# rongzhao-zhang/EfficientQ

Hardware: AMD Instinct MI355X
Metric: ptq_calibration_throughput (higher is better)
Workload: dtype i8xi8->i32 (exact) for the Gram systems and per-iteration loss convs of the layers with quantised input, f32/f64 elsewhere

## Files before the change

efficientq_amd/csrc/admm_run.hip:

```cpp
#include <stdlib.h>
#include <algorithm>
#include <vector>
#include "common.h"
#include "internal.h"
#include "project_dual.h"

namespace effq {

struct ProfRec {
  int kind, iter, loss_kind, c2, n;
  effq_geom geom;
  hipEvent_t e0, e1;
};
static thread_local std::vector<ProfRec> g_prof;
static thread_local int g_prof_every = 0;
enum { PROF_PROX = 1, PROF_FIXED_POINT = 2, PROF_PROJECT = 3, PROF_LOSS = 4, PROF_INVERSE = 5, PROF_WAIT = 6 };

struct ProfScope {
  bool on;
  hipStream_t stream;
  ProfRec rec;
  ProfScope(bool enabled, int kind, int iter, const effq_admm_run_args* a, hipStream_t st) : on(enabled), stream(st) {
    if (!on) return;
    rec.kind = kind;
// ... 239 lines not shown
};

static int enqueue_later_inverses(const effq_admm_run_args* a, const AdmmPlan& p, EventPool& events, hipEvent_t* ev_inv) {
  for (int r = p.first + 1; r < p.rhos.count; ++r) {
    float* dst = a->ainv_pool + (size_t)(r - p.first) * p.ainv_elems;
    const bool on2 = p.two_sides && ((r - p.first) % 2 == 0);
    hipStream_t sr = on2 ? p.s_side2 : p.s_side;
    void* ws = !p.fork_side ? a->inv_ws : (on2 ? a->inv_ws_side2 : a->inv_ws_side);
    const size_t wsb = !p.fork_side ? a->inv_ws_bytes : (on2 ? a->inv_ws_side2_bytes : a->inv_ws_side_bytes);
    ProfScope ps(g_prof_every > 0, PROF_INVERSE, -1 - r, a, sr);
    const int rc = effq_spd_inverse(a->A0, p.n, p.has_b, p.rhos.rho[r], a->eta, dst, ws, wsb, sr);
    if (rc != EFFQ_OK) return rc;
    ps.close();
    if (p.fork_side) {
      EFFQ_HIP(events.take(&ev_inv[r]));
      EFFQ_HIP(hipEventRecord(ev_inv[r], sr));
    }
  }
  return EFFQ_OK;
}

struct AdmmIter {
  int i;
  double rho, rho_next;
  float dual_div;
  bool use_shift, use_traj, prof;
  bool next_rhs;
  const float* G_prev;
  float *G, *bstar;
  int8_t* Gq;
  effq_fp_state* st;
  const float* parts;
  int parts_n, parts_ld;
};
static AdmmIter admm_iter(const effq_admm_run_args* a, const AdmmPlan& p, int i, double rho, bool use_traj) {
  const bool step = i % a->rho_period == 0, doubles = rho * 2 <= a->rho_max;
  const bool use_shift = p.rhos.shifted_first && i == 0;
  const bool prof = g_prof_every > 0 && !use_shift && (i % g_prof_every) == g_prof_every / 2;
  return AdmmIter{i, rho, !step ? rho : doubles ? rho * 2 : a->rho_max,
                  !step ? 1.0f : doubles ? 2.0f : (float)(a->rho_max / rho), use_shift, use_traj, prof, i + 1 < a->iters,
                  (i == 0) ? a->W0 : a->G_ring + (size_t)(i - 1) * p.nw, a->G_ring + (size_t)i * p.nw,
                  p.has_b ? a->b_ring + (size_t)i * p.c2 : nullptr, a->Gq_ring ? a->Gq_ring + (size_t)i * p.nw : nullptr,
                  a->state_ring + i, nullptr, 1, 0};
}

static int enqueue_prox(const effq_admm_run_args* a, const AdmmPlan& p, AdmmIter* it, const float* Ainv, bool bm_ready) {
  if (!it->use_shift && bm_ready && it->use_traj && p.c2 <= 512)
    return effq_prox_solve_prebuilt_parts(a->B0, Ainv, a->W0, a->b0, it->G_prev, a->dual, p.c2, p.n, p.has_b, it->rho,
                                          a->eta, a->wstar, it->bstar, a->prox_ws, a->prox_ws_bytes, p.s_main,
                                          &it->parts, &it->parts_n, &it->parts_ld);
  if (it->use_shift)
    return effq_prox_solve_shifted(a->B0, a->ainv_pool, a->W0, a->b0, it->G_prev, a->dual, p.c2, p.n, p.has_b, it->rho,
                                   a->eta, p.rhos.rho[1], shift_terms(it->rho, a->eta, p.rhos.rho[1]), a->wstar, it->bstar,
                                   a->prox_ws, a->prox_ws_bytes, p.s_main);
  const auto solve = bm_ready ? effq_prox_solve_prebuilt : effq_prox_solve;
  return solve(a->B0, Ainv, a->W0, a->b0, it->G_prev, a->dual, p.c2, p.n, p.has_b, it->rho, a->eta, a->wstar, it->bstar,
               a->prox_ws, a->prox_ws_bytes, p.s_main);
}

enum class FpKind { channels, traj, bucket, small, coop };
static FpKind fp_kind(const AdmmPlan& p, bool use_traj) {
  if (p.chan) return FpKind::channels;
  if (use_traj) return FpKind::traj;
  if (p.bucket) return FpKind::bucket;
  return p.nw <= effq_fp_small_max() ? FpKind::small : FpKind::coop;
}

static int enqueue_fixed_point(const effq_admm_run_args* a, const AdmmPlan& p, const AdmmIter& it, bool* bm_ready) {
  const int nwrow = p.n - p.has_b;
  ProjNext nx;
  memset(&nx, 0, sizeof(nx));
  if (it.next_rhs) nx = ProjNext{p.bm, a->B0, a->W0, nwrow, p.n, p.bm_ld, (float)it.rho_next, (float)a->eta};
  const ProjNext* nxp = it.next_rhs ? &nx : nullptr;
  const FpKind kind = fp_kind(p, it.use_traj);
  const bool fuse_proj = kind == FpKind::channels ||
                         (kind == FpKind::small && proj_vec_ok(a->v, a->wstar, it.G, a->dual, it.Gq, p.nw, nxp));
  ProjFused pf;
  memset(&pf, 0, sizeof(pf));
  pf.wstar = a->wstar; pf.G = it.G; pf.dual = a->dual; pf.Gq = it.Gq; pf.err_flag = a->err_flag;
  pf.d = 2.0 / (double)(a->w_levels - 1); pf.dual_div = it.dual_div; pf.lm1 = a->w_levels - 1;
  pf.n4 = (unsigned)(p.nw / 4);
  pf.nx = nx;
  void* rec = p.traj ? a->fp_pred : nullptr;
  const int maxit = 100 * a->w_levels;
  ProfScope p_fp(it.prof, PROF_FIXED_POINT, it.i, a, p.s_main);
  int rc;
  if (kind == FpKind::channels)
    rc = effq_fixed_point_channels_proj(a->wstar, a->dual, a->v, p.c2, nwrow, a->w_levels, a->tol, maxit,
                                        a->alpha_ring + (size_t)it.i * p.c2,
                                        a->w_iters_ring ? a->w_iters_ring + (size_t)it.i * p.c2 : nullptr, a->err_flag,
                                        it.G, it.dual_div, it.next_rhs ? p.bm : nullptr, a->B0, a->W0, p.n, p.bm_ld,
                                        it.rho_next, a->eta, p.s_main);
  else if (kind == FpKind::traj && it.parts != nullptr)
    rc = effq_fixed_point_traj_parts(it.parts, it.parts_n, it.parts_ld, p.c2, nwrow, p.has_b, a->dual, a->wstar, it.bstar,
                                     a->v, a->w_levels, -1.0, 1.0, a->tol, maxit, it.st, a->fp_pred, a->fp_traj_ws,
                                     a->fp_traj_ws_bytes, p.s_main);
  else if (kind == FpKind::traj)
    rc = effq_fixed_point_traj(a->wstar, a->dual, a->v, p.nw, a->w_levels, -1.0, 1.0, a->tol, maxit, it.st, a->fp_pred,
                               a->fp_traj_ws, a->fp_traj_ws_bytes, p.s_main);
  else if (kind == FpKind::bucket)
    rc = effq_fixed_point_bucket_rec(a->wstar, a->dual, a->v, p.nw, a->w_levels, -1.0, 1.0, a->tol, maxit, it.st, a->fp_ws,
                                     a->fp_ws_bytes, rec, p.s_main);
  else if (kind == FpKind::small)
    rc = effq_fixed_point_small_fused(a->wstar, a->dual, a->v, p.nw, a->w_levels, -1.0, 1.0, a->tol, maxit, it.st,
                                      fuse_proj ? &pf : nullptr, p.s_main);
  else
    rc = effq_fixed_point_coop_rec(a->wstar, a->dual, a->v, p.nw, a->w_levels, -1.0, 1.0, a->tol, maxit, it.st, a->red_ws,
                                   rec, p.s_main);
  if (rc != EFFQ_OK) return rc;
  p_fp.close();
  *bm_ready = it.next_rhs;
  if (fuse_proj) return EFFQ_OK;
  ProfScope p_pr(it.prof, PROF_PROJECT, it.i, a, p.s_main);
  rc = effq_project_dual_impl(a->v, a->wstar, it.st, a->w_levels, it.G, a->dual, it.dual_div, it.Gq, p.nw, a->err_flag,
                              nxp, p.s_main);
  if (rc != EFFQ_OK) return rc;
  p_pr.close();
  return EFFQ_OK;
}

static int enqueue_losses(const effq_admm_run_args* a, const AdmmPlan& p, int j0, int i) {
  const int step = a->loss_kind == 5 ? 16 : 1;
  for (int j = j0; j <= i; j += step) {
    const int cnt = (i - j + 1 < step) ? (i - j + 1) : step;
    const float* Gj = a->G_ring + (size_t)j * p.nw;
    const int8_t* Gqj = a->Gq_ring ? a->Gq_ring + (size_t)j * p.nw : nullptr;
    const float* bj = p.has_b ? a->b_ring + (size_t)j * p.c2 : nullptr;
    const effq_fp_state* stj = a->state_ring + j;
    double* sq = a->hist + 2 * (size_t)j;
    const bool prof = g_prof_every > 0 && (a->loss_kind == 5 ? (j / p.loss_group) % 2 == 1 :
                      !(p.rhos.shifted_first && j == 0) && (j % g_prof_every) == g_prof_every / 2);
    ProfScope p_loss(prof, PROF_LOSS, j, a, p.s_loss);
    int rc;
    if (a->loss_kind == 5)
      rc = effq_gram_loss_i8(a->loss_planes, a->loss_nplanes, a->loss_Au, a->loss_Bu, a->loss_syy, Gqj, bj, stj,
// ... 49 lines not shown
    hipEvent_t ev_fork;
    EFFQ_HIP(events.take(&ev_fork));
    EFFQ_HIP(hipEventRecord(ev_fork, p.s_main));
    EFFQ_HIP(hipStreamWaitEvent(p.s_side, ev_fork, 0));
    if (p.two_sides) EFFQ_HIP(hipStreamWaitEvent(p.s_side2, ev_fork, 0));
  }
  ProfScope p_inv(g_prof_every > 0, PROF_INVERSE, -1, a, p.s_main);
  if (const int rc = effq_spd_inverse(a->A0, p.n, p.has_b, p.rhos.rho[p.first], a->eta, a->ainv_pool, a->inv_ws,
                                      a->inv_ws_bytes, p.s_main); rc != EFFQ_OK)
    return rc;
  p_inv.close();
  if (p.fork_loss)
    for (int e = 0; e < LOSS_EVENTS; ++e) EFFQ_HIP(events.take(&ev_loss[e]));
  bool bm_ready = false;
  const float* Ainv = nullptr;
  int k = 0;
  int cur = -1;
  int loss_next = 0;
  for (int i = 0; i < a->iters; ++i) {
    if (k + 1 < p.rhos.count && p.rhos.first_iter[k + 1] == i) ++k;
    if (i == p.side_iter)
      if (const int rc = enqueue_later_inverses(a, p, events, ev_inv); rc != EFFQ_OK) return rc;
    AdmmIter it = admm_iter(a, p, i, p.rhos.rho[k], p.traj && i - p.rhos.first_iter[k] >= p.traj_after);
    if (!it.use_shift && cur != k) {
      EFFQ_CHECK_ARG(p.rhos.rho[k] == p.rhos.rho[k]);
      if (p.fork_side && ev_inv[k] != nullptr) {
        ProfScope p_wait(g_prof_every > 0, PROF_WAIT, i, a, p.s_main);
        EFFQ_HIP(hipStreamWaitEvent(p.s_main, ev_inv[k], 0));
        p_wait.close();
      }
      Ainv = a->ainv_pool + (size_t)(k - p.first) * p.ainv_elems;
      cur = k;
    }
    ProfScope p_prox(it.prof, PROF_PROX, i, a, p.s_main);
    if (const int rc = enqueue_prox(a, p, &it, Ainv, bm_ready); rc != EFFQ_OK) return rc;
    p_prox.close();
    if (const int rc = enqueue_fixed_point(a, p, it, &bm_ready); rc != EFFQ_OK) return rc;
    if (a->res_ring != nullptr) {
      const size_t nb = std::min<size_t>((p.nw + 1023) / 1024, 256);
      hipLaunchKernelGGL(k_admm_residuals, dim3((unsigned)nb), dim3(256), 0, p.s_main, a->wstar, it.G, it.G_prev, p.nw,
                         a->res_ring + 2 * (size_t)i);
      EFFQ_LAUNCH_CHECK();
    }
    if (!p.fork_loss || (i + 1) % p.loss_group == 0 || i + 1 == a->iters) {
      if (p.fork_loss) EFFQ_HIP(events.hand_over(p.s_main, p.s_loss, ev_loss[(i / p.loss_group) % LOSS_EVENTS]));
      if (const int rc = enqueue_losses(a, p, loss_next, i); rc != EFFQ_OK) return rc;
      loss_next = i + 1;
    }
  }
  ProfScope p_join(g_prof_every > 0 && (p.fork_loss || p.fork_side), PROF_WAIT, a->iters, a, p.s_main);
  if (p.fork_loss) EFFQ_HIP(events.hand_over(p.s_loss, p.s_main));
  if (p.fork_side && p.n_inv > 1) EFFQ_HIP(events.hand_over(p.s_side, p.s_main));
  if (p.fork_side && p.n_inv > 1 && p.two_sides) EFFQ_HIP(events.hand_over(p.s_side2, p.s_main));
  p_join.close();
  return EFFQ_OK;
}

size_t effq_gram_packed_elems(int n, int c2) {
  return (n > 0 && c2 > 0) ? (size_t)n * (n + 1) / 2 + (size_t)c2 * n : 0;
}

int effq_gram_pack(const float* A0, const float* B0, int n, int c2, float* buf, void* stream) {
  EFFQ_CHECK_ARG(A0 && B0 && buf && n > 0 && c2 > 0);
  size_t blocks = ((size_t)n * n + (size_t)c2 * n + 255) / 256;
  if (blocks > 8192) blocks = 8192;
  hipLaunchKernelGGL(k_gram_pack, dim3((unsigned)blocks), dim3(256), 0, as_stream(stream), A0, B0, n, c2, buf);
  EFFQ_LAUNCH_CHECK();
  return EFFQ_OK;
}
// ... 51 lines not shown
```

efficientq_amd/csrc/fixed_point_values.hip:

```cpp
#include "common.h"
#include "fp_level.h"
#include "internal.h"
#include "project_dual.h"

namespace effq {

constexpr int FPS_T = 1024;
template <int T, int PER>
__global__ __launch_bounds__(T) void k_fp_small(const float* __restrict__ a, const float* b2, float* v_out, size_t n,
                                                effq_fp_state* st, double lo, double hi, double d, double tol,
                                                int max_iter, ProjFused pf) {
  constexpr int NW = T / 64;
  __shared__ double part[2][3][NW];
  __builtin_amdgcn_s_setprio(3);
  const int tid = threadIdx.x, lane = tid & 63, wid = tid >> 6;
  const int kmax = (int)((n + T - 1) / T);
  float vr[PER];
  unsigned live = 0;
  double acc0 = 0.0, acc1 = 0.0;
#pragma unroll
  for (int k = 0; k < PER; ++k) {
    const size_t i = (size_t)tid + (size_t)k * T;
    float v = 0.0f;
    if (i < n) {
      v = (b2 != nullptr) ? (a[i] + b2[i]) : a[i];
      if (v_out != nullptr) v_out[i] = v;
      live |= 1u << k;
    }
    vr[k] = v;
    acc0 += fabs((double)v);
    acc1 += (double)v;
  }
  acc0 = wave_sum_f64_dpp(acc0);
  acc1 = wave_sum_f64_dpp(acc1);
  if (lane == 0) {
    part[0][0][wid] = acc0;
    part[0][1][wid] = acc1;
  }
  lds_barrier();
  double tot = 0.0, sv = 0.0;
#pragma unroll
  for (int w = 0; w < NW; ++w) {
    tot += part[0][0][w];
    sv += part[0][1][w];
  }
  double alpha = tot / (double)n, alpha_prev = -999.0;
  double ralpha = (double)n / tot;
  double last0 = 0.0, last1 = 0.0;
  int it = 0, done = 0;
  const double rd = 1.0 / d;
  LevelConsts lc = level_grid(lo, hi, d);
  while (!done) {
    const int par = (it + 1) & 1;
    lc.c1 = (float)(ralpha * rd);
    double arv = 0.0;
    int sr = 0, sr2 = 0;
#pragma unroll
    for (int k = 0; k < PER; ++k) {
// ... 187 lines not shown
      fpc_publish(&partials[(par * FPC_MAXG + wg) * 3 + 1], dr);
      fpc_publish(&partials[(par * FPC_MAXG + wg) * 3 + 2], dr2);
    }
    if (!fpc_barrier(counter, (++epoch) * (unsigned)G, &s_fail, spin_limit)) {
      if (tid == 0) st->done = 3;
      return;
    }
    double trv = 0.0, tr = 0.0, tr2 = 0.0;
    combine(par, trv, tr, tr2);
    const double t0 = level_sum_bv(trv, sv, lo, d);
    const double t1 = level_sum_bb(tr2, tr, n, lo, d);
    const double a_new = t0 / t1;
    alpha_prev = alpha;
    ++it;
    fp_stop(it, max_iter, a_new, alpha_prev, tol, done);
    alpha = a_new;
    last0 = t0;
    last1 = t1;
  }
  if (wg == 0 && tid == 0) fp_state_finish(st, pred, alpha, alpha_prev, last0, last1, it, done, tot, levels);
  if (tid == 0) {
    const unsigned left = __hip_atomic_fetch_add(counter + 1, 1u, __ATOMIC_RELAXED, __HIP_MEMORY_SCOPE_AGENT);
    if (left == (unsigned)G - 1) {
      __hip_atomic_store(counter, 0u, __ATOMIC_RELAXED, __HIP_MEMORY_SCOPE_AGENT);
      __hip_atomic_store(counter + 1, 0u, __ATOMIC_RELAXED, __HIP_MEMORY_SCOPE_AGENT);
    }
  }
}

__global__ void k_check_state(const effq_fp_state* st, int32_t* err_flag) {
  if (st->done != 1) *err_flag = (st->done == 2) ? 2 : 3;
}

}

using namespace effq;

extern "C" {

size_t effq_fp_small_max(void) { return (size_t)1 << 15; }

int effq_fixed_point_small(const float* a, const float* b, float* v_out, size_t n, int levels, double lo, double hi,
                           double tol, int max_iter, effq_fp_state* state_dev, void* stream) {
  return effq_fixed_point_small_fused(a, b, v_out, n, levels, lo, hi, tol, max_iter, state_dev, nullptr, stream);
}

int effq_fixed_point_small_fused(const float* a, const float* b, float* v_out, size_t n, int levels, double lo, double hi,
                                 double tol, int max_iter, effq_fp_state* state_dev, const ProjFused* pf_in, void* stream) {
  ProjFused pf;
  memset(&pf, 0, sizeof(pf));
  if (pf_in != nullptr) pf = *pf_in;
  EFFQ_CHECK_ARG(pf.G == nullptr || v_out != nullptr);
  EFFQ_CHECK_ARG(a && state_dev && n > 0 && levels >= 2 && levels <= FP_LEVELS_MAX && hi > lo && max_iter > 0);
  EFFQ_CHECK_ARG(n <= effq_fp_small_max());
  EFFQ_CHECK_ARG(b == nullptr || v_out != nullptr);
  const double d = (hi - lo) / (double)(levels - 1);
  {
    const int T = (n <= 2048) ? 256 : (n <= 16384) ? 512 : FPS_T;
    int per = (int)((n + T - 1) / T), pp = 1;
    while (pp < per) pp <<= 1;
    hipStream_t st = as_stream(stream);
#define EFFQ_FPS(TT, PP)                                                                                          \
  hipLaunchKernelGGL((k_fp_small<TT, PP>), dim3(1), dim3(TT), 0, st, a, b, v_out, n, state_dev, lo, hi, d, tol, max_iter, pf)
    if (T == 256) {
      switch (pp) {
        case 1: EFFQ_FPS(256, 1); break;
        case 2: EFFQ_FPS(256, 2); break;
        case 4: EFFQ_FPS(256, 4); break;
        case 8: EFFQ_FPS(256, 8); break;
        case 16: EFFQ_FPS(256, 16); break;
        default: EFFQ_FPS(256, 32); break;
      }
    } else if (T == 512) {
      switch (pp) {
        case 1: case 2: case 4: EFFQ_FPS(512, 4); break;
        case 8: EFFQ_FPS(512, 8); break;
        case 16: EFFQ_FPS(512, 16); break;
        default: EFFQ_FPS(512, 32); break;
      }
    } else {
      if (pp <= 16) EFFQ_FPS(1024, 16); else EFFQ_FPS(1024, 32);
    }
#undef EFFQ_FPS
  }
  EFFQ_LAUNCH_CHECK();
  return EFFQ_OK;
}

size_t effq_fp_coop_max(void) { return (size_t)FPC_SLICE * FPC_MAXG; }

int effq_fp_coop_set_spin_limit(unsigned int polls) {
  g_fpc_spin_limit = polls ? polls : FPC_SPIN_LIMIT;
  return EFFQ_OK;
}

int effq_fixed_point_coop(const float* a, const float* b, float* v_out, size_t n, int levels, double lo, double hi,
                          double tol, int max_iter, effq_fp_state* state_dev, void* ws, void* stream) {
  return effq_fixed_point_coop_rec(a, b, v_out, n, levels, lo, hi, tol, max_iter, state_dev, ws, nullptr, stream);
}

int effq_fixed_point_coop_rec(const float* a, const float* b, float* v_out, size_t n, int levels, double lo, double hi,
                              double tol, int max_iter, effq_fp_state* state_dev, void* ws, void* pred_dev,
                              void* stream) {
  FptPred* pred = reinterpret_cast<FptPred*>(pred_dev);
  EFFQ_CHECK_ARG(a && state_dev && ws && n > 0 && levels >= 2 && levels <= FP_LEVELS_MAX && hi > lo && max_iter > 0);
  EFFQ_CHECK_ARG(n <= effq_fp_coop_max());
  EFFQ_CHECK_ARG(b == nullptr || v_out != nullptr);
  EFFQ_CHECK_ARG(v_out == nullptr || (v_out != a && v_out != b));
  const double d = (hi - lo) / (double)(levels - 1);
  int G = (int)((n + FPC_SLICE - 1) / FPC_SLICE);
  if (G < 1) G = 1;
  EFFQ_CHECK_ARG(G <= FPC_MAXG);
  const size_t per = (n + G - 1) / G;
  const size_t lds = per * sizeof(float);
  double* partials = reinterpret_cast<double*>(ws);
  unsigned int* counter = reinterpret_cast<unsigned int*>(reinterpret_cast<char*>(ws) +
                                                          sizeof(double) * RED_MAX_BLOCKS * RED_SLOTS + 64);
  hipStream_t st = as_stream(stream);
  int dev = 0;
// ... 36 lines not shown
```

efficientq_amd/csrc/internal.h:

```cpp
#pragma once
#include "common.h"

namespace effq {
struct ProjFused;
struct ProjNext;
}

extern "C" {

int effq_fixed_point_small_fused(const float* a, const float* b, float* v_out, size_t n, int levels, double lo, double hi,
                                 double tol, int max_iter, effq_fp_state* state_dev, const effq::ProjFused* pf_in,
                                 void* stream);
int effq_project_dual_impl(const float* v, const float* wstar, const effq_fp_state* state_dev, int levels, float* G,
                           float* dual, float dual_div, int8_t* Gq_out, size_t n, int32_t* err_flag_dev,
                           const effq::ProjNext* nx, void* stream);

float* effq_prox_bm(void* ws, int c2, int n, int* ldb);
int effq_prox_solve_prebuilt(const float* B0, const float* Ainv, const float* W0, const float* b0, const float* G,
                             const float* dual, int c2, int n, int has_bias, double rho, double eta, float* wstar,
                             float* bstar, void* ws, size_t ws_bytes, void* stream);
int effq_prox_solve_prebuilt_parts(const float* B0, const float* Ainv, const float* W0, const float* b0, const float* G,
                                   const float* dual, int c2, int n, int has_bias, double rho, double eta, float* wstar,
                                   float* bstar, void* ws, size_t ws_bytes, void* stream, const float** part_out,
                                   int* nsplit_out, int* ldp_out);

int effq_fixed_point_traj_parts(const float* part, int nsplit, int ldp, int c2, int nwrow, int has_bias, const float* dual,
                                float* wstar_out, float* bstar_out, float* v_out, int levels, double lo, double hi, double tol,
                                int max_iter, effq_fp_state* state_dev, void* pred_dev, void* ws, size_t ws_bytes,
                                void* stream);

}
```

efficientq_amd/csrc/solve.hip:

```cpp
#include <cstdlib>
#include <vector>
#include "common.h"
#include "internal.h"

namespace effq {

typedef float f32x16 __attribute__((ext_vector_type(16)));
typedef double f64x4 __attribute__((ext_vector_type(4)));
typedef float f32x4 __attribute__((ext_vector_type(4)));

static inline int round_up(int v, int m) { return (v + m - 1) / m * m; }

constexpr int NBK = 64;
constexpr int LDA_S = 66;
constexpr int LDB_S = 80;

__global__ __launch_bounds__(256) void k_build_a64(const float* __restrict__ A0, int n, int npad, int has_bias,
                                                   double rho, double eta, double* __restrict__ A64) {
  const size_t tot = (size_t)npad * npad;
  const size_t stride = (size_t)gridDim.x * blockDim.x;
  for (size_t e = (size_t)blockIdx.x * blockDim.x + threadIdx.x; e < tot; e += stride) {
    const int i = (int)(e / npad), j = (int)(e % npad);
    double v = 0.0;
    if (i < n && j < n) {
      v = (double)A0[(size_t)i * n + j];
      if (i == j) v += eta + ((has_bias && i == n - 1) ? 0.0 : rho);
    } else if (i == j) {
      v = 1.0;
    }
    A64[e] = v;
  }
}

__device__ __forceinline__ double readlane_f64(double v, int lane) {
  const int lo = __builtin_amdgcn_readlane(__double2loint(v), lane);
  const int hi = __builtin_amdgcn_readlane(__double2hiint(v), lane);
  return __hiloint2double(hi, lo);
}

template <int CPW>
__device__ __forceinline__ void gj_invert_regs(double (&reg)[CPW], double (*fcol)[NBK + 1], int lane, int wid) {
#pragma unroll
// ... 624 lines not shown
      }
    } else if (r < c2 && k == nw && has_bias) {
      v.x = B0[(size_t)r * n + k] + eta * b0[r];
    }
    *reinterpret_cast<float4*>(out + k) = v;
  }
}

__global__ __launch_bounds__(256) void k_prox_reduce4(const float* __restrict__ part, int ldp, int nsplit, int c2, int n,
                                                      int has_bias, float* __restrict__ wstar, float* __restrict__ bstar) {
  __builtin_amdgcn_s_setprio(2);

  const int r = blockIdx.y;
  const int nw = n - has_bias;
  const size_t tot = (size_t)c2 * ldp;
  const float* row = part + (size_t)r * ldp;
  for (int k = (blockIdx.x * blockDim.x + threadIdx.x) * 4; k < ldp; k += gridDim.x * blockDim.x * 4) {
    if (k >= n) continue;
    float4 v = *reinterpret_cast<const float4*>(row + k);
    for (int z = 1; z < nsplit; ++z) {
      const float4 t = *reinterpret_cast<const float4*>(row + (size_t)z * tot + k);
      v.x += t.x;
      v.y += t.y;
      v.z += t.z;
      v.w += t.w;
    }
    if (k < nw)
      *reinterpret_cast<float4*>(wstar + (size_t)r * nw + k) = v;
    else
      bstar[r] = v.x;
  }
}

constexpr int PBK = 32, PLD = PBK + 4;

template <int MT, int WM, int WN, int NTN>
__global__ __launch_bounds__(256) void k_prox_gemm(const float* __restrict__ Bm, int ldb, const float* __restrict__ Ainv,
                                                   int lda, int n, int c2, int has_bias, float* __restrict__ wstar,
                                                   float* __restrict__ bstar, float* __restrict__ part, int ldp) {
  __builtin_amdgcn_s_setprio(2);

  constexpr int BM = 32 * MT * WM, BN = 32 * WN * NTN;
  constexpr int NA = BM * 8 / 256, NB = BN * 8 / 256;
  static_assert(WM * WN == 4 && NA >= 1 && NB >= 1, "4 waves");
  __shared__ __attribute__((aligned(16))) float As[BM * PLD];
  __shared__ __attribute__((aligned(16))) float Bs[BN * PLD];
  const int tid = threadIdx.x, lane = tid & 63, wid = tid >> 6;
  const int li = lane & 31, lh = lane >> 5;
  const int wm = wid / WN, wn = wid % WN;
  const int row0 = blockIdx.y * BM, col0 = blockIdx.x * BN;

  f32x16 acc[MT][NTN];
#pragma unroll
  for (int m = 0; m < MT; ++m)
#pragma unroll
    for (int t = 0; t < NTN; ++t)
#pragma unroll
      for (int r = 0; r < 16; ++r) acc[m][t][r] = 0.0f;

  f32x4 ra[NA], rb[NB];
  const float* pa[NA];
  const float* pb[NB];
#pragma unroll
  for (int q = 0; q < NA; ++q) {
    const int u = tid + q * 256, r = u >> 3, c4 = u & 7;
    pa[q] = Bm + (size_t)(row0 + r) * ldb + c4 * 4;
  }
#pragma unroll
  for (int q = 0; q < NB; ++q) {
    const int u = tid + q * 256, r = u >> 3, c4 = u & 7;
    pb[q] = Ainv + (size_t)min(col0 + r, n - 1) * lda + c4 * 4;
  }
#define EFFQ_PROX_FETCH(k0)                                                         \
  {                                                                                 \
    _Pragma("unroll") for (int q = 0; q < NA; ++q)                                  \
        ra[q] = *reinterpret_cast<const f32x4*>(pa[q] + (k0));                      \
    _Pragma("unroll") for (int q = 0; q < NB; ++q)                                  \
        rb[q] = *reinterpret_cast<const f32x4*>(pb[q] + (k0));                      \
  }
  const int nkt = ldb / PBK;
  const int kt0 = (int)(((long long)nkt * blockIdx.z) / gridDim.z);
  const int nk = (int)(((long long)nkt * (blockIdx.z + 1)) / gridDim.z);
  EFFQ_PROX_FETCH(kt0 * PBK)
  for (int kt = kt0; kt < nk; ++kt) {
    lds_barrier();
#pragma unroll
    for (int q = 0; q < NA; ++q) {
      const int u = tid + q * 256;
      *reinterpret_cast<f32x4*>(&As[(u >> 3) * PLD + (u & 7) * 4]) = ra[q];
    }
#pragma unroll
    for (int q = 0; q < NB; ++q) {
      const int u = tid + q * 256;
      *reinterpret_cast<f32x4*>(&Bs[(u >> 3) * PLD + (u & 7) * 4]) = rb[q];
    }
    lds_barrier();
    EFFQ_PROX_FETCH(min(kt + 1, nk - 1) * PBK)
    __builtin_amdgcn_sched_barrier(0);
#pragma unroll
    for (int q = 0; q < 4; ++q) {
      f32x4 a[MT], b[NTN];
#pragma unroll
      for (int m = 0; m < MT; ++m)
        a[m] = *reinterpret_cast<const f32x4*>(&As[((wm * MT + m) * 32 + li) * PLD + q * 8 + 4 * lh]);
#pragma unroll
      for (int t = 0; t < NTN; ++t)
        b[t] = *reinterpret_cast<const f32x4*>(&Bs[((wn * NTN + t) * 32 + li) * PLD + q * 8 + 4 * lh]);
#pragma unroll
      for (int m = 0; m < MT; ++m)
#pragma unroll
        for (int t = 0; t < NTN; ++t)
#pragma unroll
          for (int e = 0; e < 4; ++e)
            acc[m][t] = __builtin_amdgcn_mfma_f32_32x32x2f32(a[m][e], b[t][e], acc[m][t], 0, 0, 0);
    }
  }
#undef EFFQ_PROX_FETCH
  const int nw = n - has_bias;
  if (gridDim.z > 1) {
    float* P = part + (size_t)blockIdx.z * c2 * ldp;
#pragma unroll
    for (int m = 0; m < MT; ++m)
#pragma unroll
      for (int t = 0; t < NTN; ++t) {
        const int col = col0 + (wn * NTN + t) * 32 + li;
#pragma unroll
        for (int r = 0; r < 16; ++r) {
          const int row = row0 + (wm * MT + m) * 32 + (r & 3) + 8 * (r >> 2) + 4 * lh;
          if (row < c2 && col < n) P[(size_t)row * ldp + col] = acc[m][t][r];
        }
      }
    return;
  }
#pragma unroll
  for (int m = 0; m < MT; ++m)
#pragma unroll
    for (int t = 0; t < NTN; ++t) {
      const int col = col0 + (wn * NTN + t) * 32 + li;
#pragma unroll
      for (int r = 0; r < 16; ++r) {
        const int row = row0 + (wm * MT + m) * 32 + (r & 3) + 8 * (r >> 2) + 4 * lh;
        if (row < c2 && col < n) {
          if (col < nw)
            wstar[(size_t)row * nw + col] = acc[m][t][r];
          else
            bstar[row] = acc[m][t][r];
        }
      }
    }
}


typedef __bf16 bf16x8 __attribute__((ext_vector_type(8)));
typedef __bf16 bf16x4 __attribute__((ext_vector_type(4)));
constexpr int B3_K = 16;
constexpr int B3_LD = B3_K + 8;

__device__ __forceinline__ void split3(const f32x4 v, bf16x4& p0, bf16x4& p1, bf16x4& p2) {
#pragma unroll
  for (int e = 0; e < 4; ++e) {
    const __bf16 b0 = (__bf16)v[e];
    const float r1 = v[e] - (float)b0;
    const __bf16 b1 = (__bf16)r1;
    const float r2 = r1 - (float)b1;
    p0[e] = b0;
    p1[e] = b1;
    p2[e] = (__bf16)r2;
  }
}

template <int BM, int BN, int WM, int WN>
__global__ __launch_bounds__(512) void k_prox_gemm_b3(const float* __restrict__ Bm, int ldb, const float* __restrict__ Ainv,
                                                      int lda, int n, int c2, int has_bias, float* __restrict__ wstar,
                                                      float* __restrict__ bstar, float* __restrict__ part, int ldp) {
  __builtin_amdgcn_s_setprio(2);
  constexpr int MT = BM / WM / 32, NT = BN / WN / 32;
  constexpr int NA = BM * 4 / 512, NB = BN * 4 / 512;
  constexpr int STAGE = 3 * (BM + BN) * B3_LD;
  static_assert(WM * WN == 8 && MT >= 1 && NT >= 1 && NA >= 1 && NB >= 1, "8 waves");
  extern __shared__ __attribute__((aligned(16))) unsigned char b3_lds[];
  __bf16* lds = reinterpret_cast<__bf16*>(b3_lds);
  const int tid = threadIdx.x, lane = tid & 63, wid = tid >> 6;
// ... 497 lines not shown
```

Measured before the change: 25.38.

## Fuse single-tile prox GEMM into small fixed-point kernel to drop a launch

For small layers whose prox GEMM fits in one block, the MFMA GEMM tile now runs at the start of the single-block fixed-point kernel instead of as a separate kernel launch. When the fixed-point kernel has more than 256 threads, the extra threads mirror the GEMM's LDS barriers so they stay in step. The GEMM body moves into a shared header so both kernels can use it. This saves one kernel launch and one global round-trip per ADMM iteration, at the cost of more LDS and register pressure in the fixed-point kernel, and it only applies to a narrow set of shapes.

After: 25.44, median of 5. Within noise of the previous version (+0.2%).

```diff
diff --git a/efficientq_amd/csrc/admm_run.hip b/efficientq_amd/csrc/admm_run.hip
--- a/efficientq_amd/csrc/admm_run.hip
+++ b/efficientq_amd/csrc/admm_run.hip
@@ -295,6 +295,8 @@
   effq_fp_state* st;
   const float* parts;
   int parts_n, parts_ld;
+  const float* Ainv;
+  bool fuse_prox;
 };
 static AdmmIter admm_iter(const effq_admm_run_args* a, const AdmmPlan& p, int i, double rho, bool use_traj) {
   const bool step = i % a->rho_period == 0, doubles = rho * 2 <= a->rho_max;
@@ -304,7 +306,7 @@
                   !step ? 1.0f : doubles ? 2.0f : (float)(a->rho_max / rho), use_shift, use_traj, prof, i + 1 < a->iters,
                   (i == 0) ? a->W0 : a->G_ring + (size_t)(i - 1) * p.nw, a->G_ring + (size_t)i * p.nw,
                   p.has_b ? a->b_ring + (size_t)i * p.c2 : nullptr, a->Gq_ring ? a->Gq_ring + (size_t)i * p.nw : nullptr,
-                  a->state_ring + i, nullptr, 1, 0};
+                  a->state_ring + i, nullptr, 1, 0, nullptr, false};
 }
 
 static int enqueue_prox(const effq_admm_run_args* a, const AdmmPlan& p, AdmmIter* it, const float* Ainv, bool bm_ready) {
@@ -328,16 +330,24 @@
   if (p.bucket) return FpKind::bucket;
   return p.nw <= effq_fp_small_max() ? FpKind::small : FpKind::coop;
 }
+static ProjNext proj_next(const effq_admm_run_args* a, const AdmmPlan& p, const AdmmIter& it) {
+  ProjNext nx;
+  memset(&nx, 0, sizeof(nx));
+  if (it.next_rhs) nx = ProjNext{p.bm, a->B0, a->W0, p.n - p.has_b, p.n, p.bm_ld, (float)it.rho_next, (float)a->eta};
+  return nx;
+}
+static bool small_fuses_proj(const effq_admm_run_args* a, const AdmmPlan& p, const AdmmIter& it) {
+  const ProjNext nx = proj_next(a, p, it);
+  return fp_kind(p, it.use_traj) == FpKind::small &&
+         proj_vec_ok(a->v, a->wstar, it.G, a->dual, it.Gq, p.nw, it.next_rhs ? &nx : nullptr);
+}
 
 static int enqueue_fixed_point(const effq_admm_run_args* a, const AdmmPlan& p, const AdmmIter& it, bool* bm_ready) {
   const int nwrow = p.n - p.has_b;
-  ProjNext nx;
-  memset(&nx, 0, sizeof(nx));
-  if (it.next_rhs) nx = ProjNext{p.bm, a->B0, a->W0, nwrow, p.n, p.bm_ld, (float)it.rho_next, (float)a->eta};
+  const ProjNext nx = proj_next(a, p, it);
   const ProjNext* nxp = it.next_rhs ? &nx : nullptr;
   const FpKind kind = fp_kind(p, it.use_traj);
-  const bool fuse_proj = kind == FpKind::channels ||
-                         (kind == FpKind::small && proj_vec_ok(a->v, a->wstar, it.G, a->dual, it.Gq, p.nw, nxp));
+  const bool fuse_proj = kind == FpKind::channels || small_fuses_proj(a, p, it);
   ProjFused pf;
   memset(&pf, 0, sizeof(pf));
   pf.wstar = a->wstar; pf.G = it.G; pf.dual = a->dual; pf.Gq = it.Gq; pf.err_flag = a->err_flag;
@@ -364,6 +374,9 @@
   else if (kind == FpKind::bucket)
     rc = effq_fixed_point_bucket_rec(a->wstar, a->dual, a->v, p.nw, a->w_levels, -1.0, 1.0, a->tol, maxit, it.st, a->fp_ws,
                                      a->fp_ws_bytes, rec, p.s_main);
+  else if (kind == FpKind::small && it.fuse_prox)
+    rc = effq_fixed_point_small_prox(a->prox_ws, it.Ainv, p.c2, p.n, p.has_b, a->dual, a->wstar, it.bstar, a->v, a->w_levels,
+                                     -1.0, 1.0, a->tol, maxit, it.st, &pf, p.s_main);
   else if (kind == FpKind::small)
     rc = effq_fixed_point_small_fused(a->wstar, a->dual, a->v, p.nw, a->w_levels, -1.0, 1.0, a->tol, maxit, it.st,
                                       fuse_proj ? &pf : nullptr, p.s_main);
@@ -479,9 +492,14 @@
       Ainv = a->ainv_pool + (size_t)(k - p.first) * p.ainv_elems;
       cur = k;
     }
-    ProfScope p_prox(it.prof, PROF_PROX, i, a, p.s_main);
-    if (const int rc = enqueue_prox(a, p, &it, Ainv, bm_ready); rc != EFFQ_OK) return rc;
-    p_prox.close();
+    it.fuse_prox = !it.use_shift && bm_ready && small_fuses_proj(a, p, it) &&
+                   effq_fixed_point_small_prox_ok(p.c2, p.n, p.has_b) != 0;
+    it.Ainv = Ainv;
+    if (!it.fuse_prox) {
+      ProfScope p_prox(it.prof, PROF_PROX, i, a, p.s_main);
+      if (const int rc = enqueue_prox(a, p, &it, Ainv, bm_ready); rc != EFFQ_OK) return rc;
+      p_prox.close();
+    }
     if (const int rc = enqueue_fixed_point(a, p, it, &bm_ready); rc != EFFQ_OK) return rc;
     if (a->res_ring != nullptr) {
       const size_t nb = std::min<size_t>((p.nw + 1023) / 1024, 256);
diff --git a/efficientq_amd/csrc/fixed_point_values.hip b/efficientq_amd/csrc/fixed_point_values.hip
--- a/efficientq_amd/csrc/fixed_point_values.hip
+++ b/efficientq_amd/csrc/fixed_point_values.hip
@@ -2,18 +2,41 @@
 #include "fp_level.h"
 #include "internal.h"
 #include "project_dual.h"
+#include "prox_gemm.h"
 
 namespace effq {
 
 constexpr int FPS_T = 1024;
-template <int T, int PER>
+struct ProxTile {
+  const float* Bm;
+  const float* Ainv;
+  int ldb, lda, n, c2, has_bias;
+  float* wstar;
+  float* bstar;
+};
+template <int T, int PER, int GEMM>
 __global__ __launch_bounds__(T) void k_fp_small(const float* __restrict__ a, const float* b2, float* v_out, size_t n,
                                                 effq_fp_state* st, double lo, double hi, double d, double tol,
-                                                int max_iter, ProjFused pf) {
+                                                int max_iter, ProjFused pf, const ProxTile pt) {
   constexpr int NW = T / 64;
   __shared__ double part[2][3][NW];
   __builtin_amdgcn_s_setprio(3);
   const int tid = threadIdx.x, lane = tid & 63, wid = tid >> 6;
+  const float* aw = a;
+  if constexpr (GEMM != 0) {
+    if (T == 256 || tid < 256) {
+      if constexpr (GEMM == 2)
+        prox_gemm_tile<1, 2, 2, 1>(pt.Bm, pt.ldb, pt.Ainv, pt.lda, pt.n, pt.c2, pt.has_bias, pt.wstar, pt.bstar, nullptr,
+                                   pt.ldb);
+      else
+        prox_gemm_tile<1, 1, 4, 1>(pt.Bm, pt.ldb, pt.Ainv, pt.lda, pt.n, pt.c2, pt.has_bias, pt.wstar, pt.bstar, nullptr,
+                                   pt.ldb);
+    } else {
+      prox_gemm_tile_wait(pt.ldb);
+    }
+    __syncthreads();
+    aw = pt.wstar;
+  }
   const int kmax = (int)((n + T - 1) / T);
   float vr[PER];
   unsigned live = 0;
@@ -23,7 +46,7 @@
     const size_t i = (size_t)tid + (size_t)k * T;
     float v = 0.0f;
     if (i < n) {
-      v = (b2 != nullptr) ? (a[i] + b2[i]) : a[i];
+      v = (b2 != nullptr) ? (aw[i] + b2[i]) : aw[i];
       if (v_out != nullptr) v_out[i] = v;
       live |= 1u << k;
     }
@@ -277,6 +300,73 @@
   if (st->done != 1) *err_flag = (st->done == 2) ? 2 : 3;
 }
 
+static void fps_shape(size_t n, int* T, int* slots) {
+  *T = (n <= 2048) ? 256 : (n <= 16384) ? 512 : FPS_T;
+  const int per = (int)((n + *T - 1) / *T);
+  int pw = 1;
+  while (pw < per) pw <<= 1;
+  if (pw > 32) pw = 32;
+  if (*T == 512 && pw < 4) pw = 4;
+  if (*T == FPS_T && pw < 16) pw = 16;
+  *slots = pw;
+}
+static bool fps_gemm_instance(int variant, int T, int slots) {
+  if (variant == 2) return T == 256 && slots == 8;
+  return variant == 3 && ((T == 256 && (slots == 1 || slots == 8)) || (T == 512 && slots == 8));
+}
+
+static int fps_launch(const float* a, const float* b, float* v_out, size_t n, int levels, double lo, double hi, double tol,
+                      int max_iter, effq_fp_state* state_dev, const ProjFused* pf_in, void* stream, const ProxTile* pt_in,
+                      int variant) {
+  ProjFused pf;
+  memset(&pf, 0, sizeof(pf));
+  if (pf_in != nullptr) pf = *pf_in;
+  ProxTile pt;
+  memset(&pt, 0, sizeof(pt));
+  if (pt_in != nullptr) pt = *pt_in;
+  EFFQ_CHECK_ARG(pf.G == nullptr || v_out != nullptr);
+  EFFQ_CHECK_ARG(state_dev && n > 0 && levels >= 2 && levels <= FP_LEVELS_MAX && hi > lo && max_iter > 0);
+  EFFQ_CHECK_ARG(n <= effq_fp_small_max());
+  EFFQ_CHECK_ARG(b == nullptr || v_out != nullptr);
+  const double d = (hi - lo) / (double)(levels - 1);
+  int T, slots;
+  fps_shape(n, &T, &slots);
+  hipStream_t st = as_stream(stream);
+#define EFFQ_FPS_AS(TT, PP, GEMM)                                                                                    \
+  hipLaunchKernelGGL((k_fp_small<TT, PP, GEMM>), dim3(1), dim3(TT), 0, st, a, b, v_out, n, state_dev, lo, hi, d, tol, \
+                     max_iter, pf, pt)
+#define EFFQ_FPS(TT, PP) EFFQ_FPS_AS(TT, PP, 0)
+  if (pt_in != nullptr) {
+    EFFQ_CHECK_ARG(fps_gemm_instance(variant, T, slots));
+    if (variant == 2) EFFQ_FPS_AS(256, 8, 2);
+    else if (T == 512) EFFQ_FPS_AS(512, 8, 3);
+    else if (slots == 8) EFFQ_FPS_AS(256, 8, 3);
+    else EFFQ_FPS_AS(256, 1, 3);
+  } else if (T == 256) {
+    switch (slots) {
+      case 1: EFFQ_FPS(256, 1); break;
+      case 2: EFFQ_FPS(256, 2); break;
+      case 4: EFFQ_FPS(256, 4); break;
+      case 8: EFFQ_FPS(256, 8); break;
+      case 16: EFFQ_FPS(256, 16); break;
+      default: EFFQ_FPS(256, 32); break;
+    }
+  } else if (T == 512) {
+    switch (slots) {
+      case 4: EFFQ_FPS(512, 4); break;
+      case 8: EFFQ_FPS(512, 8); break;
+      case 16: EFFQ_FPS(512, 16); break;
+      default: EFFQ_FPS(512, 32); break;
+    }
+  } else {
+    if (slots <= 16) EFFQ_FPS(1024, 16); else EFFQ_FPS(1024, 32);
+  }
+#undef EFFQ_FPS
+#undef EFFQ_FPS_AS
+  EFFQ_LAUNCH_CHECK();
+  return EFFQ_OK;
+}
+
 }
 
 using namespace effq;
@@ -292,44 +382,32 @@
 
 int effq_fixed_point_small_fused(const float* a, const float* b, float* v_out, size_t n, int levels, double lo, double hi,
                                  double tol, int max_iter, effq_fp_state* state_dev, const ProjFused* pf_in, void* stream) {
-  ProjFused pf;
-  memset(&pf, 0, sizeof(pf));
-  if (pf_in != nullptr) pf = *pf_in;
-  EFFQ_CHECK_ARG(pf.G == nullptr || v_out != nullptr);
-  EFFQ_CHECK_ARG(a && state_dev && n > 0 && levels >= 2 && levels <= FP_LEVELS_MAX && hi > lo && max_iter > 0);
-  EFFQ_CHECK_ARG(n <= effq_fp_small_max());
-  EFFQ_CHECK_ARG(b == nullptr || v_out != nullptr);
-  const double d = (hi - lo) / (double)(levels - 1);
-  {
-    const int T = (n <= 2048) ? 256 : (n <= 16384) ? 512 : FPS_T;
-    int per = (int)((n + T - 1) / T), pp = 1;
-    while (pp < per) pp <<= 1;
-    hipStream_t st = as_stream(stream);
-#define EFFQ_FPS(TT, PP)                                                                                          \
-  hipLaunchKernelGGL((k_fp_small<TT, PP>), dim3(1), dim3(TT), 0, st, a, b, v_out, n, state_dev, lo, hi, d, tol, max_iter, pf)
-    if (T == 256) {
-      switch (pp) {
-        case 1: EFFQ_FPS(256, 1); break;
-        case 2: EFFQ_FPS(256, 2); break;
-        case 4: EFFQ_FPS(256, 4); break;
-        case 8: EFFQ_FPS(256, 8); break;
-        case 16: EFFQ_FPS(256, 16); break;
-        default: EFFQ_FPS(256, 32); break;
-      }
-    } else if (T == 512) {
-      switch (pp) {
-        case 1: case 2: case 4: EFFQ_FPS(512, 4); break;
-        case 8: EFFQ_FPS(512, 8); break;
-        case 16: EFFQ_FPS(512, 16); break;
-        default: EFFQ_FPS(512, 32); break;
-      }
-    } else {
-      if (pp <= 16) EFFQ_FPS(1024, 16); else EFFQ_FPS(1024, 32);
-    }
-#undef EFFQ_FPS
-  }
-  EFFQ_LAUNCH_CHECK();
-  return EFFQ_OK;
+  EFFQ_CHECK_ARG(a != nullptr);
+  return fps_launch(a, b, v_out, n, levels, lo, hi, tol, max_iter, state_dev, pf_in, stream, nullptr, -1);
+}
+
+int effq_fixed_point_small_prox_ok(int c2, int n, int has_bias) {
+  int variant = 0, gx = 0, gy = 0, nsplit = 0, T = 0, slots = 0;
+  if (c2 <= 0 || n <= 1 || effq_prox_plan_query(c2, n, &variant, &gx, &gy, &nsplit) != EFFQ_OK) return 0;
+  const size_t nw = (size_t)c2 * (size_t)(n - (has_bias ? 1 : 0));
+  if (gx * gy * nsplit != 1 || nw > effq_fp_small_max()) return 0;
+  fps_shape(nw, &T, &slots);
+  return fps_gemm_instance(variant, T, slots) ? 1 : 0;
+}
+
+int effq_fixed_point_small_prox(void* prox_ws, const float* Ainv, int c2, int n, int has_bias, const float* dual,
+                                float* wstar_out, float* bstar_out, float* v_out, int levels, double lo, double hi, double tol,
+                                int max_iter, effq_fp_state* state_dev, const ProjFused* pf_in, void* stream) {
+  EFFQ_CHECK_ARG(prox_ws && Ainv && dual && wstar_out && v_out && (!has_bias || bstar_out != nullptr));
+  EFFQ_CHECK_ARG(v_out != wstar_out && v_out != dual && effq_fixed_point_small_prox_ok(c2, n, has_bias));
+  int variant = 0, gx = 0, gy = 0, nsplit = 0;
+  EFFQ_CHECK_ARG(effq_prox_plan_query(c2, n, &variant, &gx, &gy, &nsplit) == EFFQ_OK);
+  ProxTile pt;
+  pt.Bm = effq_prox_bm(prox_ws, c2, n, &pt.ldb);
+  pt.Ainv = Ainv; pt.lda = effq_ainv_ld(n); pt.n = n; pt.c2 = c2; pt.has_bias = has_bias ? 1 : 0;
+  pt.wstar = wstar_out; pt.bstar = has_bias ? bstar_out : nullptr;
+  return fps_launch(nullptr, dual, v_out, (size_t)c2 * (size_t)(n - pt.has_bias), levels, lo, hi, tol, max_iter, state_dev,
+                    pf_in, stream, &pt, variant);
 }
 
 size_t effq_fp_coop_max(void) { return (size_t)FPC_SLICE * FPC_MAXG; }
diff --git a/efficientq_amd/csrc/internal.h b/efficientq_amd/csrc/internal.h
--- a/efficientq_amd/csrc/internal.h
+++ b/efficientq_amd/csrc/internal.h
@@ -29,4 +29,9 @@
                                 int max_iter, effq_fp_state* state_dev, void* pred_dev, void* ws, size_t ws_bytes,
                                 void* stream);
 
+int effq_fixed_point_small_prox_ok(int c2, int n, int has_bias);
+int effq_fixed_point_small_prox(void* prox_ws, const float* Ainv, int c2, int n, int has_bias, const float* dual,
+                                float* wstar_out, float* bstar_out, float* v_out, int levels, double lo, double hi, double tol,
+                                int max_iter, effq_fp_state* state_dev, const effq::ProjFused* pf_in, void* stream);
+
 }
diff --git a/efficientq_amd/csrc/prox_gemm.h b/efficientq_amd/csrc/prox_gemm.h
--- /dev/null
+++ b/efficientq_amd/csrc/prox_gemm.h
@@ -0,0 +1,132 @@
+#pragma once
+#include "common.h"
+
+namespace effq {
+
+typedef float f32x4 __attribute__((ext_vector_type(4)));
+typedef float f32x16 __attribute__((ext_vector_type(16)));
+
+constexpr int PBK = 32, PLD = PBK + 4;
+
+template <int MT, int WM, int WN, int NTN>
+__device__ __forceinline__ void prox_gemm_tile(const float* __restrict__ Bm, int ldb, const float* __restrict__ Ainv,
+                                               int lda, int n, int c2, int has_bias, float* __restrict__ wstar,
+                                               float* __restrict__ bstar, float* __restrict__ part, int ldp) {
+  constexpr int BM = 32 * MT * WM, BN = 32 * WN * NTN;
+  constexpr int NA = BM * 8 / 256, NB = BN * 8 / 256;
+  static_assert(WM * WN == 4 && NA >= 1 && NB >= 1, "4 waves");
+  __shared__ __attribute__((aligned(16))) float As[BM * PLD];
+  __shared__ __attribute__((aligned(16))) float Bs[BN * PLD];
+  const int tid = threadIdx.x, lane = tid & 63, wid = tid >> 6;
+  const int li = lane & 31, lh = lane >> 5;
+  const int wm = wid / WN, wn = wid % WN;
+  const int row0 = blockIdx.y * BM, col0 = blockIdx.x * BN;
+
+  f32x16 acc[MT][NTN];
+#pragma unroll
+  for (int m = 0; m < MT; ++m)
+#pragma unroll
+    for (int t = 0; t < NTN; ++t)
+#pragma unroll
+      for (int r = 0; r < 16; ++r) acc[m][t][r] = 0.0f;
+
+  f32x4 ra[NA], rb[NB];
+  const float* pa[NA];
+  const float* pb[NB];
+#pragma unroll
+  for (int q = 0; q < NA; ++q) {
+    const int u = tid + q * 256, r = u >> 3, c4 = u & 7;
+    pa[q] = Bm + (size_t)(row0 + r) * ldb + c4 * 4;
+  }
+#pragma unroll
+  for (int q = 0; q < NB; ++q) {
+    const int u = tid + q * 256, r = u >> 3, c4 = u & 7;
+    pb[q] = Ainv + (size_t)min(col0 + r, n - 1) * lda + c4 * 4;
+  }
+#define EFFQ_PROX_FETCH(k0)                                                         \
+  {                                                                                 \
+    _Pragma("unroll") for (int q = 0; q < NA; ++q)                                  \
+        ra[q] = *reinterpret_cast<const f32x4*>(pa[q] + (k0));                      \
+    _Pragma("unroll") for (int q = 0; q < NB; ++q)                                  \
+        rb[q] = *reinterpret_cast<const f32x4*>(pb[q] + (k0));                      \
+  }
+  const int nkt = ldb / PBK;
+  const int kt0 = (int)(((long long)nkt * blockIdx.z) / gridDim.z);
+  const int nk = (int)(((long long)nkt * (blockIdx.z + 1)) / gridDim.z);
+  EFFQ_PROX_FETCH(kt0 * PBK)
+  for (int kt = kt0; kt < nk; ++kt) {
+    lds_barrier();
+#pragma unroll
+    for (int q = 0; q < NA; ++q) {
+      const int u = tid + q * 256;
+      *reinterpret_cast<f32x4*>(&As[(u >> 3) * PLD + (u & 7) * 4]) = ra[q];
+    }
+#pragma unroll
+    for (int q = 0; q < NB; ++q) {
+      const int u = tid + q * 256;
+      *reinterpret_cast<f32x4*>(&Bs[(u >> 3) * PLD + (u & 7) * 4]) = rb[q];
+    }
+    lds_barrier();
+    EFFQ_PROX_FETCH(min(kt + 1, nk - 1) * PBK)
+    __builtin_amdgcn_sched_barrier(0);
+#pragma unroll
+    for (int q = 0; q < 4; ++q) {
+      f32x4 a[MT], b[NTN];
+#pragma unroll
+      for (int m = 0; m < MT; ++m)
+        a[m] = *reinterpret_cast<const f32x4*>(&As[((wm * MT + m) * 32 + li) * PLD + q * 8 + 4 * lh]);
+#pragma unroll
+      for (int t = 0; t < NTN; ++t)
+        b[t] = *reinterpret_cast<const f32x4*>(&Bs[((wn * NTN + t) * 32 + li) * PLD + q * 8 + 4 * lh]);
+#pragma unroll
+      for (int m = 0; m < MT; ++m)
+#pragma unroll
+        for (int t = 0; t < NTN; ++t)
+#pragma unroll
+          for (int e = 0; e < 4; ++e)
+            acc[m][t] = __builtin_amdgcn_mfma_f32_32x32x2f32(a[m][e], b[t][e], acc[m][t], 0, 0, 0);
+    }
+  }
+#undef EFFQ_PROX_FETCH
+  const int nw = n - has_bias;
+  if (gridDim.z > 1) {
+    float* P = part + (size_t)blockIdx.z * c2 * ldp;
+#pragma unroll
+    for (int m = 0; m < MT; ++m)
+#pragma unroll
+      for (int t = 0; t < NTN; ++t) {
+        const int col = col0 + (wn * NTN + t) * 32 + li;
+#pragma unroll
+        for (int r = 0; r < 16; ++r) {
+          const int row = row0 + (wm * MT + m) * 32 + (r & 3) + 8 * (r >> 2) + 4 * lh;
+          if (row < c2 && col < n) P[(size_t)row * ldp + col] = acc[m][t][r];
+        }
+      }
+    return;
+  }
+#pragma unroll
+  for (int m = 0; m < MT; ++m)
+#pragma unroll
+    for (int t = 0; t < NTN; ++t) {
+      const int col = col0 + (wn * NTN + t) * 32 + li;
+#pragma unroll
+      for (int r = 0; r < 16; ++r) {
+        const int row = row0 + (wm * MT + m) * 32 + (r & 3) + 8 * (r >> 2) + 4 * lh;
+        if (row < c2 && col < n) {
+          if (col < nw)
+            wstar[(size_t)row * nw + col] = acc[m][t][r];
+          else
+            bstar[row] = acc[m][t][r];
+        }
+      }
+    }
+}
+
+__device__ __forceinline__ void prox_gemm_tile_wait(int ldb) {
+  for (int kt = 0; kt < ldb / PBK; ++kt) {
+    lds_barrier();
+    lds_barrier();
+  }
+}
+
+}
diff --git a/efficientq_amd/csrc/solve.hip b/efficientq_amd/csrc/solve.hip
--- a/efficientq_amd/csrc/solve.hip
+++ b/efficientq_amd/csrc/solve.hip
@@ -2,12 +2,11 @@
 #include <vector>
 #include "common.h"
 #include "internal.h"
+#include "prox_gemm.h"
 
 namespace effq {
 
-typedef float f32x16 __attribute__((ext_vector_type(16)));
 typedef double f64x4 __attribute__((ext_vector_type(4)));
-typedef float f32x4 __attribute__((ext_vector_type(4)));
 
 static inline int round_up(int v, int m) { return (v + m - 1) / m * m; }
 
@@ -698,122 +697,13 @@
   }
 }
 
-constexpr int PBK = 32, PLD = PBK + 4;
-
 template <int MT, int WM, int WN, int NTN>
 __global__ __launch_bounds__(256) void k_prox_gemm(const float* __restrict__ Bm, int ldb, const float* __restrict__ Ainv,
                                                    int lda, int n, int c2, int has_bias, float* __restrict__ wstar,
                                                    float* __restrict__ bstar, float* __restrict__ part, int ldp) {
   __builtin_amdgcn_s_setprio(2);
 
-  constexpr int BM = 32 * MT * WM, BN = 32 * WN * NTN;
-  constexpr int NA = BM * 8 / 256, NB = BN * 8 / 256;
-  static_assert(WM * WN == 4 && NA >= 1 && NB >= 1, "4 waves");
-  __shared__ __attribute__((aligned(16))) float As[BM * PLD];
-  __shared__ __attribute__((aligned(16))) float Bs[BN * PLD];
-  const int tid = threadIdx.x, lane = tid & 63, wid = tid >> 6;
-  const int li = lane & 31, lh = lane >> 5;
-  const int wm = wid / WN, wn = wid % WN;
-  const int row0 = blockIdx.y * BM, col0 = blockIdx.x * BN;
-
-  f32x16 acc[MT][NTN];
-#pragma unroll
-  for (int m = 0; m < MT; ++m)
-#pragma unroll
-    for (int t = 0; t < NTN; ++t)
-#pragma unroll
-      for (int r = 0; r < 16; ++r) acc[m][t][r] = 0.0f;
-
-  f32x4 ra[NA], rb[NB];
-  const float* pa[NA];
-  const float* pb[NB];
-#pragma unroll
-  for (int q = 0; q < NA; ++q) {
-    const int u = tid + q * 256, r = u >> 3, c4 = u & 7;
-    pa[q] = Bm + (size_t)(row0 + r) * ldb + c4 * 4;
-  }
-#pragma unroll
-  for (int q = 0; q < NB; ++q) {
-    const int u = tid + q * 256, r = u >> 3, c4 = u & 7;
-    pb[q] = Ainv + (size_t)min(col0 + r, n - 1) * lda + c4 * 4;
-  }
-#define EFFQ_PROX_FETCH(k0)                                                         \
-  {                                                                                 \
-    _Pragma("unroll") for (int q = 0; q < NA; ++q)                                  \
-        ra[q] = *reinterpret_cast<const f32x4*>(pa[q] + (k0));                      \
-    _Pragma("unroll") for (int q = 0; q < NB; ++q)                                  \
-        rb[q] = *reinterpret_cast<const f32x4*>(pb[q] + (k0));                      \
-  }
-  const int nkt = ldb / PBK;
-  const int kt0 = (int)(((long long)nkt * blockIdx.z) / gridDim.z);
-  const int nk = (int)(((long long)nkt * (blockIdx.z + 1)) / gridDim.z);
-  EFFQ_PROX_FETCH(kt0 * PBK)
-  for (int kt = kt0; kt < nk; ++kt) {
-    lds_barrier();
-#pragma unroll
-    for (int q = 0; q < NA; ++q) {
-      const int u = tid + q * 256;
-      *reinterpret_cast<f32x4*>(&As[(u >> 3) * PLD + (u & 7) * 4]) = ra[q];
-    }
-#pragma unroll
-    for (int q = 0; q < NB; ++q) {
-      const int u = tid + q * 256;
-      *reinterpret_cast<f32x4*>(&Bs[(u >> 3) * PLD + (u & 7) * 4]) = rb[q];
-    }
-    lds_barrier();
-    EFFQ_PROX_FETCH(min(kt + 1, nk - 1) * PBK)
-    __builtin_amdgcn_sched_barrier(0);
-#pragma unroll
-    for (int q = 0; q < 4; ++q) {
-      f32x4 a[MT], b[NTN];
-#pragma unroll
-      for (int m = 0; m < MT; ++m)
-        a[m] = *reinterpret_cast<const f32x4*>(&As[((wm * MT + m) * 32 + li) * PLD + q * 8 + 4 * lh]);
-#pragma unroll
-      for (int t = 0; t < NTN; ++t)
-        b[t] = *reinterpret_cast<const f32x4*>(&Bs[((wn * NTN + t) * 32 + li) * PLD + q * 8 + 4 * lh]);
-#pragma unroll
-      for (int m = 0; m < MT; ++m)
-#pragma unroll
-        for (int t = 0; t < NTN; ++t)
-#pragma unroll
-          for (int e = 0; e < 4; ++e)
-            acc[m][t] = __builtin_amdgcn_mfma_f32_32x32x2f32(a[m][e], b[t][e], acc[m][t], 0, 0, 0);
-    }
-  }
-#undef EFFQ_PROX_FETCH
-  const int nw = n - has_bias;
-  if (gridDim.z > 1) {
-    float* P = part + (size_t)blockIdx.z * c2 * ldp;
-#pragma unroll
-    for (int m = 0; m < MT; ++m)
-#pragma unroll
-      for (int t = 0; t < NTN; ++t) {
-        const int col = col0 + (wn * NTN + t) * 32 + li;
-#pragma unroll
-        for (int r = 0; r < 16; ++r) {
-          const int row = row0 + (wm * MT + m) * 32 + (r & 3) + 8 * (r >> 2) + 4 * lh;
-          if (row < c2 && col < n) P[(size_t)row * ldp + col] = acc[m][t][r];
-        }
-      }
-    return;
-  }
-#pragma unroll
-  for (int m = 0; m < MT; ++m)
-#pragma unroll
-    for (int t = 0; t < NTN; ++t) {
-      const int col = col0 + (wn * NTN + t) * 32 + li;
-#pragma unroll
-      for (int r = 0; r < 16; ++r) {
-        const int row = row0 + (wm * MT + m) * 32 + (r & 3) + 8 * (r >> 2) + 4 * lh;
-        if (row < c2 && col < n) {
-          if (col < nw)
-            wstar[(size_t)row * nw + col] = acc[m][t][r];
-          else
-            bstar[row] = acc[m][t][r];
-        }
-      }
-    }
+  prox_gemm_tile<MT, WM, WN, NTN>(Bm, ldb, Ainv, lda, n, c2, has_bias, wstar, bstar, part, ldp);
 }
 
 
```
